# hugofloresgarcia/vampnet

Measured on NVIDIA H100. Metric: codec tokens/sec (coarse 12 steps + c2f 24 steps generate, T=768, 44.1 kHz), higher is better.
Workload: dtype bf16

## Files before the change

vampnet_b200/csrc/api.cu:

```cuda
#include <cuda_bf16.h>
#include <cudaTypedefs.h>

#include <cmath>
#include <cstdarg>
#include <cstdio>
#include <cstring>
#include <map>
#include <memory>
#include <string>
#include <tuple>
#include <vector>

#include "kernels.h"

namespace vnb {

static thread_local std::string g_err;
static thread_local std::string g_tmap_err;

static int fail(const char* fmt, ...) {
  char buf[1024];
  va_list ap;
  va_start(ap, fmt);
  vsnprintf(buf, sizeof(buf), fmt, ap);
// ... 27 lines not shown
  auto enc = get_encode();
  if (!enc) return false;
  cuuint64_t dims[2] = {cols, rows};
  cuuint64_t strides[1] = {cols * 2};
  cuuint32_t box[2] = {box_cols, box_rows};
  cuuint32_t estr[2] = {1, 1};
  CUresult r = enc(tm, CU_TENSOR_MAP_DATA_TYPE_BFLOAT16, 2, const_cast<void*>(base), dims, strides, box, estr,
                   CU_TENSOR_MAP_INTERLEAVE_NONE, CU_TENSOR_MAP_SWIZZLE_128B, CU_TENSOR_MAP_L2_PROMOTION_L2_256B,
                   CU_TENSOR_MAP_FLOAT_OOB_FILL_NONE);
  if (r != CUDA_SUCCESS) {
    char b[256];
    snprintf(b, sizeof(b), "cuTensorMapEncodeTiled(2d rows=%llu cols=%llu box=%ux%u) -> %d", (unsigned long long)rows,
             (unsigned long long)cols, box_rows, box_cols, (int)r);
    g_tmap_err = b;
    return false;
  }
  return true;
}
bool make_tmap_3d(CUtensorMap* tm, const void* base, uint64_t batch, uint64_t rows, uint64_t cols,
                  uint64_t pitch_elems, uint32_t box_rows, uint32_t box_cols) {
  auto enc = get_encode();
  if (!enc) return false;
  cuuint64_t dims[3] = {cols, rows, batch};
  cuuint64_t strides[2] = {pitch_elems * 2, rows * pitch_elems * 2};
  cuuint32_t box[3] = {box_cols, box_rows, 1};
  cuuint32_t estr[3] = {1, 1, 1};
  CUresult r = enc(tm, CU_TENSOR_MAP_DATA_TYPE_BFLOAT16, 3, const_cast<void*>(base), dims, strides, box, estr,
                   CU_TENSOR_MAP_INTERLEAVE_NONE, CU_TENSOR_MAP_SWIZZLE_128B, CU_TENSOR_MAP_L2_PROMOTION_L2_256B,
                   CU_TENSOR_MAP_FLOAT_OOB_FILL_NONE);
  if (r != CUDA_SUCCESS) {
    char b[256];
    snprintf(b, sizeof(b), "cuTensorMapEncodeTiled(3d batch=%llu rows=%llu cols=%llu pitch=%llu box=%ux%u) -> %d",
             (unsigned long long)batch, (unsigned long long)rows, (unsigned long long)cols,
             (unsigned long long)pitch_elems, box_rows, box_cols, (int)r);
    g_tmap_err = b;
    return false;
  }
  return true;
}

static bool make_gemm_plan(GemmPlan* p, int epi, const void* A, const void* W, int M, int N, int K, void* out,
                           void* out2, const float* bias, int T, int Tpad, const float* ss_in, int ss_parts,
                           float inv_d, float eps, void* out_bf16, float* ss_out) {
  if (N % 256 != 0 || K % 64 != 0 || M < 1) {
    g_tmap_err = "gemm: need N % 256 == 0 and K % 64 == 0";
    return false;
  }
  GemmArgs& a = p->args;
  a.M = M; a.N = N; a.K = K; a.epi = epi; a.out = out; a.out2 = out2; a.bias = bias;
  a.T = T; a.Tpad = Tpad; a.d2 = epi == VNB_EPI_QKV ? (N / 3) * 2 : 0;
  if (ss_in != nullptr) { a.ss_in = ss_in; a.ss_parts = ss_parts; a.inv_d = inv_d; a.eps = eps; }
  a.out_bf16 = reinterpret_cast<__nv_bfloat16*>(out_bf16); a.ss_out = ss_out;
  return make_tmap_2d(&p->tmA, A, M, K, 128, 64) && make_tmap_2d(&p->tmB, W, N, K, 256, 64) &&
         make_tmap_2d(&p->tmBh, W, N, K, 128, 64);
}

bool make_attn_plan(AttnPlan* p, const void* qk, const void* vT, void* out, const float* rel, int sat, int B, int T,
                    int Tpad, int H) {
  const int d = H * 64;
  p->out = out; p->rel = rel; p->sat = sat; p->B = B; p->T = T; p->Tpad = Tpad; p->H = H;
  return make_tmap_3d(&p->tmQ, qk, B, T, 2 * d, 2 * d, 128, 64) && make_tmap_3d(&p->tmK, qk, B, T, 2 * d, 2 * d, 64, 64) &&
         make_tmap_3d(&p->tmVT, vT, B, d, Tpad, Tpad, 64, 64);
}

struct DevBuf {
  void* p = nullptr;
  size_t n = 0;
  ~DevBuf() { if (p) cudaFree(p); }
  cudaError_t alloc(size_t bytes, bool zero = false) {
    n = bytes;
    cudaError_t e = cudaMalloc(&p, bytes ? bytes : 1);
    if (e == cudaSuccess && zero) e = cudaMemset(p, 0, bytes);
    return e;
  }
  template <class T> T* as() const { return reinterpret_cast<T*>(p); }
};

struct Variant {
  int steps = 0;
  bool has_mask = false;
  bool top_p = false;
  int gemm_pair = 0;
  bool fused = false;
  bool adapted = false;
  bool ragged = false;
  bool mixed_steps = false;
  bool split = false;
  bool operator<(const Variant& o) const {
    return std::tie(steps, has_mask, top_p, gemm_pair, fused, adapted, ragged, mixed_steps, split) <
           std::tie(o.steps, o.has_mask, o.top_p, o.gemm_pair, o.fused, o.adapted, o.ragged, o.mixed_steps, o.split);
  }
};

struct Workspace {
  int B = 0, T = 0, Tpad = 0, M = 0;
  unsigned long long last_use = 0;
  DevBuf x, y, qk, vT, att, h, logits, zcur, zorig, tokens, conf, n0, dyn, rowgrp, z_in, mask_in, z_out, ssA, ssB, embA,
      partials;
  DevBuf grp_adapter, lora_u;
  DevBuf frames;
  DevBuf live;
  int embKp = 0;
  int ss_parts = 0;
  std::vector<GemmPlan> qkv, wo, up, down;
  GemmPlan cls, emb;
  GemmPlan cls_sample;
  bool can_fuse = false;
// ... 1161 lines not shown
```

vampnet_b200/csrc/common.cuh:

```cuda
#pragma once
#include <cuda.h>
#include <cuda_bf16.h>
#include <cuda_runtime.h>
#include <stdint.h>
#include <stdio.h>

namespace vnb {

__device__ __forceinline__ uint32_t smem_u32(const void* p) {
  return static_cast<uint32_t>(__cvta_generic_to_shared(p));
}
__device__ __forceinline__ uint32_t lane_id() { return threadIdx.x & 31; }

__device__ __forceinline__ bool elect_one() {
  uint32_t pred = 0;
  asm volatile(
      "{\n\t.reg .pred P;\n\t.reg .b32 R;\n\t"
      "elect.sync R|P, 0xffffffff;\n\t"
      "selp.u32 %0, 1, 0, P;\n\t}"
      : "=r"(pred));
  return pred != 0;
}

__device__ __forceinline__ void mbar_init(uint64_t* bar, uint32_t count) {
// ... 121 lines not shown
  asm volatile(
      "{\n\t.reg .pred P;\n\t"
      "mbarrier.try_wait.parity.acquire.cluster.shared::cta.b64 P, [%1], %2, %3;\n\t"
      "selp.u32 %0, 1, 0, P;\n\t}"
      : "=r"(ok)
      : "r"(smem_u32(bar)), "r"(parity), "r"(100000u)
      : "memory");
  return ok != 0;
}
__device__ __forceinline__ void mbar_wait_cluster(uint64_t* bar, uint32_t parity) {
  if (mbar_try_wait_cluster(bar, parity)) return;
  const uint64_t t0 = global_timer_ns();
  while (!mbar_try_wait_cluster(bar, parity))
    if (global_timer_ns() - t0 > VNB_WAIT_TIMEOUT_NS) __trap();
}
__device__ __forceinline__ void tma_load_2d_mc(void* dst, const CUtensorMap* m, uint64_t* bar, int c0, int c1,
                                               uint16_t cta_mask) {
  asm volatile(
      "cp.async.bulk.tensor.2d.shared::cluster.global.mbarrier::complete_tx::bytes.multicast::cluster"
      " [%0], [%1, {%3, %4}], [%2], %5;"
      ::"r"(smem_u32(dst)), "l"(reinterpret_cast<uint64_t>(m)), "r"(smem_u32(bar)), "r"(c0), "r"(c1), "h"(cta_mask)
      : "memory");
}

__device__ __forceinline__ uint32_t pack_bf16x2(float lo, float hi) {
  __nv_bfloat162 v = __floats2bfloat162_rn(lo, hi);
  return *reinterpret_cast<uint32_t*>(&v);
}
__device__ __forceinline__ float fast_exp2(float x) {
  float y;
  asm volatile("ex2.approx.ftz.f32 %0, %1;" : "=f"(y) : "f"(x));
  return y;
}
__device__ __forceinline__ float lds_f32(uint32_t addr) {
  float v;
  asm volatile("ld.shared.f32 %0, [%1];" : "=f"(v) : "r"(addr));
  return v;
}
__device__ __forceinline__ void sts_f32(uint32_t addr, float v) {
  asm volatile("st.shared.f32 [%0], %1;" ::"r"(addr), "f"(v) : "memory");
}
__device__ __forceinline__ void sts_u32(uint32_t addr, uint32_t v) {
  asm volatile("st.shared.b32 [%0], %1;" ::"r"(addr), "r"(v) : "memory");
}
__device__ __forceinline__ float4 lds_f4(uint32_t addr) {
  float4 v;
  asm volatile("ld.shared.v4.f32 {%0, %1, %2, %3}, [%4];" : "=f"(v.x), "=f"(v.y), "=f"(v.z), "=f"(v.w) : "r"(addr));
  return v;
}
__device__ __forceinline__ uint2 lds_u2(uint32_t addr) {
  uint2 v;
  asm volatile("ld.shared.v2.b32 {%0, %1}, [%2];" : "=r"(v.x), "=r"(v.y) : "r"(addr));
  return v;
}
__device__ __forceinline__ void sts_f4(uint32_t addr, float4 v) {
  asm volatile("st.shared.v4.f32 [%0], {%1, %2, %3, %4};" ::"r"(addr), "f"(v.x), "f"(v.y), "f"(v.z), "f"(v.w)
               : "memory");
}
__device__ __forceinline__ void sts_v4(uint32_t addr, uint32_t a, uint32_t b, uint32_t c, uint32_t d) {
  asm volatile("st.shared.v4.b32 [%0], {%1, %2, %3, %4};" ::"r"(addr), "r"(a), "r"(b), "r"(c), "r"(d) : "memory");
}
__device__ __forceinline__ float warp_max(float v) {
#pragma unroll
  for (int o = 16; o > 0; o >>= 1) v = fmaxf(v, __shfl_xor_sync(0xffffffffu, v, o));
  return v;
}
__device__ __forceinline__ float warp_sum(float v) {
#pragma unroll
  for (int o = 16; o > 0; o >>= 1) v += __shfl_xor_sync(0xffffffffu, v, o);
  return v;
}

__device__ __forceinline__ void philox4x32_10(uint32_t c0, uint32_t c1, uint32_t c2, uint32_t c3, uint32_t k0,
                                              uint32_t k1, uint32_t (&out)[4]) {
#pragma unroll
  for (int r = 0; r < 10; ++r) {
    const uint32_t hi0 = __umulhi(0xD2511F53u, c0), lo0 = 0xD2511F53u * c0;
    const uint32_t hi1 = __umulhi(0xCD9E8D57u, c2), lo1 = 0xCD9E8D57u * c2;
    const uint32_t n0 = hi1 ^ c1 ^ k0, n2 = hi0 ^ c3 ^ k1;
    c0 = n0; c1 = lo1; c2 = n2; c3 = lo0;
    k0 += 0x9E3779B9u;
    k1 += 0xBB67AE85u;
  }
  out[0] = c0; out[1] = c1; out[2] = c2; out[3] = c3;
}
__device__ __forceinline__ float u01(uint32_t x) { return (static_cast<float>(x >> 9) + 0.5f) * 1.1920928955078125e-07f; }

}
```

vampnet_b200/csrc/gemm_wgmma.cu:

```cuda
#include <stdlib.h>

#include "common.cuh"
#include "kernels.h"
#include "wgmma.cuh"

#ifndef VNB_GEMM_PAIR_DEFAULT
#define VNB_GEMM_PAIR_DEFAULT false
#endif

namespace vnb {

constexpr int BM = 128, BN = 256, BK = 64, STAGES = 4;
constexpr int A_BYTES = BM * BK * 2;
constexpr int B_BYTES = BN * BK * 2;
constexpr int STAGE_BYTES = A_BYTES + B_BYTES;
constexpr int SBIAS_BYTES = BN * 4;
constexpr int RING_BYTES = STAGES * STAGE_BYTES;
constexpr int ACC_PITCH = BN + 1;
static_assert(BM * ACC_PITCH * 4 <= RING_BYTES, "the accumulator tile overlays the ring");
static_assert(BM * ACC_PITCH * 4 + 4 * BM + 16 + 32 * BM <= RING_BYTES, "the adapted epilogue's row table follows it");
constexpr int GEMM_SMEM = RING_BYTES + SBIAS_BYTES + 1024  + 256 ;
static_assert(GEMM_SMEM <= 227 * 1024, "H100: at most 227 KiB of shared memory per block");
constexpr int GEMM_THREADS = 256 + 32;
template <int EPI> constexpr int gemm_epi_warps() { return (EPI == VNB_EPI_RESID || EPI == VNB_EPI_SAMPLE) ? 8 : 4; }

__device__ __forceinline__ int live_rows(const GemmArgs& g) {
  if (g.live == nullptr) return g.M;
  const int r = __ldg(g.live) * g.T;
  return r < g.M ? r : g.M;
}

__device__ __forceinline__ float gelu_tanh(float x) {
  const float y = 0.7978845608028654f * (x + 0.044715f * x * x * x);
  const float e = __expf(2.0f * y);
  const float t = 1.0f - __fdividef(2.0f, 1.0f + e);
  return 0.5f * x * (1.0f + t);
}

__device__ __forceinline__ float row_scale(const GemmArgs& g, int row) {
  float rs = 1.0f;
  if (g.ss_in != nullptr && row < g.M) {
    float t = 0.f;
    for (int p = 0; p < g.ss_parts; ++p) t += __ldg(g.ss_in + static_cast<size_t>(p) * g.M + row);
    rs = rsqrtf(t * g.inv_d + g.eps);
  }
  return rs;
}


__device__ __forceinline__ float sumsq4(float x, float y, float z, float w) {
  return __fmaf_rn(w, w, __fmaf_rn(z, z, __fmaf_rn(y, y, __fmul_rn(x, x))));
}

template <int EPI>
__device__ __forceinline__ void prefetch_addend(const GemmArgs& g, int lane, int row_base, int col0, float4 (&add)[8]) {
  const int c4 = (lane & 7) * 4;
  const int r0 = row_base + (lane >> 3);
  if constexpr (EPI == VNB_EPI_RESID) {
    const float* base = reinterpret_cast<const float*>(g.out) + static_cast<size_t>(r0) * g.N + col0 + c4;
    const size_t step = static_cast<size_t>(4) * g.N;
#pragma unroll
    for (int it = 0; it < 8; ++it)
      add[it] = (r0 + it * 4 < g.M) ? __ldcg(reinterpret_cast<const float4*>(base + it * step))
                                    : make_float4(0.f, 0.f, 0.f, 0.f);
  } else {
    const float4 b4 = __ldg(reinterpret_cast<const float4*>(g.bias + col0 + c4));
#pragma unroll
    for (int it = 0; it < 8; ++it) add[it] = b4;
  }
}
template <bool FUSED>
__device__ __forceinline__ void drain_f32(const GemmArgs& g, uint32_t quad, float rs, int lane, int row_base, int n0,
                                          int c, const float4 (&add)[8], float (&ssacc)[8]) {
  const int c4 = (lane & 7) * 4;
  const int r0 = row_base + (lane >> 3);
  const int col0 = n0 + c * 32;
  float* const base = reinterpret_cast<float*>(g.out) + static_cast<size_t>(r0) * g.N + col0 + c4;
  const size_t step = static_cast<size_t>(4) * g.N;
#pragma unroll
  for (int it = 0; it < 8; ++it) {
    const int r = it * 4 + (lane >> 3);
    const float rsr = __shfl_sync(0xffffffffu, rs, r);
    const uint32_t sp = quad + 4u * (r * ACC_PITCH + c * 32 + c4);
    float4 a = make_float4(__fmul_rn(lds_f32(sp), rsr), __fmul_rn(lds_f32(sp + 4), rsr), __fmul_rn(lds_f32(sp + 8), rsr),
                           __fmul_rn(lds_f32(sp + 12), rsr));
    a.x = __fadd_rn(a.x, add[it].x); a.y = __fadd_rn(a.y, add[it].y);
    a.z = __fadd_rn(a.z, add[it].z); a.w = __fadd_rn(a.w, add[it].w);
    if (r0 + it * 4 < g.M) {
      *reinterpret_cast<float4*>(base + it * step) = a;
      if constexpr (FUSED) {
        uint2 w;
        w.x = pack_bf16x2(a.x, a.y);
        w.y = pack_bf16x2(a.z, a.w);
        *reinterpret_cast<uint2*>(g.out_bf16 + static_cast<size_t>(r0 + it * 4) * g.N + col0 + c4) = w;
        ssacc[it] = __fadd_rn(ssacc[it], sumsq4(a.x, a.y, a.z, a.w));
      }
    }
  }
}

template <bool GEGLU>
__device__ __forceinline__ void drain_bf16(__nv_bfloat16* out, int pitch, int M, uint32_t quad, float rs, int lane,
                                           int row_base, int tc, int oc) {
  const int c8 = (lane & 3) * 8;
#pragma unroll
  for (int it = 0; it < 4; ++it) {
    const int r = it * 8 + (lane >> 2);
    const float rsr = __shfl_sync(0xffffffffu, rs, r);
    const uint32_t sp = quad + 4u * (r * ACC_PITCH + tc + c8);
    float x[8];
#pragma unroll
    for (int k = 0; k < 8; ++k) {
      x[k] = lds_f32(sp + 4u * k) * rsr;
      if constexpr (GEGLU) x[k] = x[k] * gelu_tanh(lds_f32(sp + 4u * (128 + k)) * rsr);
    }
    const int row = row_base + r;
    if (row < M) {
      uint4 w;
      w.x = pack_bf16x2(x[0], x[1]);
      w.y = pack_bf16x2(x[2], x[3]);
      w.z = pack_bf16x2(x[4], x[5]);
      w.w = pack_bf16x2(x[6], x[7]);
      *reinterpret_cast<uint4*>(out + static_cast<size_t>(row) * pitch + oc + c8) = w;
    }
  }
}

__device__ __forceinline__ void acc_ld_x32(uint32_t addr, uint32_t (&v)[32]) {
#pragma unroll
  for (int j = 0; j < 32; ++j) v[j] = __float_as_uint(lds_f32(addr + 4u * j));
}

template <int EPI>
__device__ __forceinline__ void lora_update(const GemmArgs& g, uint8_t* scratch, uint32_t acc_tile, int m0, int n0) {
  int uoff = 0, brow0 = n0;
  if constexpr (EPI == VNB_EPI_QKV) {
    const int d = g.N / 3;
    if (n0 >= d && n0 < 2 * d) return;
    if (n0 >= 2 * d) { uoff = 8; brow0 = n0 - d; }
  }
  const AdapterRefs& L = g.lora;
  const int t = static_cast<int>(threadIdx.x);
  int32_t* sid = reinterpret_cast<int32_t*>(scratch);
  uint32_t* smask = reinterpret_cast<uint32_t*>(scratch + 4 * BM);
  float4* su = reinterpret_cast<float4*>(scratch + 4 * BM + 16);
  constexpr int R = EPI == VNB_EPI_QKV ? 16 : 8;
  if (t < BM) {
    const int m = m0 + t;
    const int id = m < g.M ? L.grp_adapter[L.rowgrp[m / L.rows_per_grp].group] : -1;
    sid[t] = id;
    if (id >= 0) {
      su[2 * t] = __ldg(reinterpret_cast<const float4*>(L.u + static_cast<size_t>(m) * R + uoff));
      su[2 * t + 1] = __ldg(reinterpret_cast<const float4*>(L.u + static_cast<size_t>(m) * R + uoff + 4));
    }
    uint32_t bits = 0;
    for (int a = 0; a < VNB_MAX_ADAPTERS; ++a) bits |= __ballot_sync(0xffffffffu, id == a) ? (1u << a) : 0u;
    if ((t & 31) == 0) smask[t >> 5] = bits;
  }
  asm volatile("bar.sync 1, 256;" ::: "memory");
  const uint32_t present = smask[0] | smask[1] | smask[2] | smask[3];
  const int nb = EPI == VNB_EPI_QKV ? 2 * (g.N / 3) : g.N;
  const int c0 = t & 63, rq = t >> 6;
  for (int a = 0; a < VNB_MAX_ADAPTERS; ++a) {
    if (!((present >> a) & 1u)) continue;
    const float* bp = L.table[a].b[L.slot] + (static_cast<size_t>(L.layer) * nb + brow0 + c0) * 8;
    float4 b0[4], b1[4];
#pragma unroll
    for (int j = 0; j < 4; ++j) {
      b0[j] = __ldg(reinterpret_cast<const float4*>(bp + 64 * 8 * j));
      b1[j] = __ldg(reinterpret_cast<const float4*>(bp + 64 * 8 * j + 4));
    }
#pragma unroll 4
    for (int i = 0; i < BM / 4; ++i) {
      const int r = rq + 4 * i;
      if (sid[r] != a) continue;
      const float4 ua = su[2 * r], ub = su[2 * r + 1];
      const uint32_t row_addr = acc_tile + 4u * (r * ACC_PITCH + c0);
#pragma unroll
      for (int j = 0; j < 4; ++j) {
        float s = __fmul_rn(ua.x, b0[j].x);
        s = __fmaf_rn(ua.y, b0[j].y, s); s = __fmaf_rn(ua.z, b0[j].z, s); s = __fmaf_rn(ua.w, b0[j].w, s);
        s = __fmaf_rn(ub.x, b1[j].x, s); s = __fmaf_rn(ub.y, b1[j].y, s); s = __fmaf_rn(ub.z, b1[j].z, s);
        s = __fmaf_rn(ub.w, b1[j].w, s);
        const uint32_t addr = row_addr + 4u * (64 * j);
        sts_f32(addr, __fadd_rn(lds_f32(addr), s));
      }
    }
  }
}

template <int NS, typename Release>
__device__ __forceinline__ void gemm_mainloop(float (&acc)[128], uint8_t* ring, uint64_t* full_bar, int num_kb, int wg,
                                              int& stage, uint32_t& phase, Release&& release) {
#pragma unroll
  for (int i = 0; i < 128; ++i) acc[i] = 0.f;
  for (int kb = 0; kb < num_kb; ++kb) {
    mbar_wait(&full_bar[stage], phase);
    const uint32_t sa = smem_u32(ring + stage * STAGE_BYTES) + wg * (64 * 128);
    const uint32_t sb = smem_u32(ring + stage * STAGE_BYTES + A_BYTES);
    wgmma_fence();
#pragma unroll
    for (int k = 0; k < BK / 16; ++k)
      wgmma_ss_n256(acc, wgmma_desc_sw128(sa + k * 32), wgmma_desc_sw128(sb + k * 32), 1u);
    wgmma_commit();
    wgmma_wait<1>();
    wgmma_fence_regs(acc);
    if (kb > 0) release(stage == 0 ? NS - 1 : stage - 1);
    if (++stage == NS) { stage = 0; phase ^= 1; }
  }
  wgmma_wait<0>();
  wgmma_fence_regs(acc);
  if (num_kb > 0) release(stage == 0 ? NS - 1 : stage - 1);
}

template <int EPI, bool PAIR, bool ADAPT = false, bool SPLIT = false>
__global__ void __launch_bounds__(GEMM_THREADS, 1)
gemm_wgmma_kernel(const __grid_constant__ CUtensorMap tmA, const __grid_constant__ CUtensorMap tmB,
                  const GemmArgs g) {
  extern __shared__ uint8_t smem_raw[];
  uint8_t* smem = reinterpret_cast<uint8_t*>((reinterpret_cast<uintptr_t>(smem_raw) + 1023) & ~uintptr_t(1023));
  float* sbias_all = reinterpret_cast<float*>(smem + RING_BYTES);
  uint64_t* full_bar = reinterpret_cast<uint64_t*>(smem + RING_BYTES + SBIAS_BYTES);
  uint64_t* empty_bar = full_bar + STAGES;

  const int warp = threadIdx.x >> 5;
  const int lane = threadIdx.x & 31;
  const uint32_t rank = PAIR ? cluster_ctarank() : 0u;
  const int tile = PAIR ? static_cast<int>(blockIdx.x >> 1) : static_cast<int>(blockIdx.x);
  constexpr int TM = PAIR ? 2 * BM : BM;
  const int num_n = g.N / BN;
  const int num_kb = g.K / BK;
  const int m0 = (tile / num_n) * TM + static_cast<int>(rank) * BM;
  const int n0 = (tile % num_n) * BN;
  if (g.live != nullptr && (tile / num_n) * TM >= live_rows(g)) return;

  if (warp == 8 && lane == 0) {
    tma_prefetch_desc(&tmA);
    tma_prefetch_desc(&tmB);
    for (int s = 0; s < STAGES; ++s) {
      mbar_init(&full_bar[s], 1);
      mbar_init(&empty_bar[s], 8 * (PAIR ? 2 : 1));
    }
    mbar_fence_init();
  }
  if constexpr (PAIR) cluster_sync_all();
  else __syncthreads();

  if (warp == 8) {
    if (lane == 0) {
      int stage = 0;
      uint32_t phase = 0;
      for (int kb = 0; kb < num_kb; ++kb) {
        if constexpr (PAIR) mbar_wait_cluster(&empty_bar[stage], phase ^ 1);
        else mbar_wait(&empty_bar[stage], phase ^ 1);
        uint8_t* sa = smem + stage * STAGE_BYTES;
        uint8_t* sb = sa + A_BYTES;
// ... 122 lines not shown
            uint32_t v[32];
            acc_ld_x32(t_strip + 4u * (c * 32), v);
#pragma unroll
            for (int j4 = 0; j4 < 8; ++j4) {
              const float4 b4 = lds_f4(sb4 + 16u * (c * 8 + j4));
              const float bj[4] = {b4.x, b4.y, b4.z, b4.w};
#pragma unroll
              for (int j = 0; j < 4; ++j) {
                const float x = __fadd_rn(__fmul_rn(__uint_as_float(v[j4 * 4 + j]), rs), bj[j]);
                ssum += fast_exp2(__fmaf_rn(x, c1, c0));
              }
            }
          }
          int cand = am;
          float xc = mx;
          if (do_sample) {
            uint32_t r4[4];
            philox4x32_10(static_cast<uint32_t>(t_idx * Cp + cp), static_cast<uint32_t>(b_idx - rg.first),
                          static_cast<uint32_t>(dyn.step), 0u, dyn.seed_lo, dyn.seed_hi, r4);
            const float target = u01(r4[1]) * ssum;
            float run = 0.f;
            int found = -1;
#pragma unroll 1
            for (int c = 0; c < 4; ++c) {
              uint32_t v[32];
              acc_ld_x32(t_strip + 4u * (c * 32), v);
#pragma unroll
              for (int j4 = 0; j4 < 8; ++j4) {
                const float4 b4 = lds_f4(sb4 + 16u * (c * 8 + j4));
                const float bj[4] = {b4.x, b4.y, b4.z, b4.w};
#pragma unroll
                for (int j = 0; j < 4; ++j) {
                  const float x = __fadd_rn(__fmul_rn(__uint_as_float(v[j4 * 4 + j]), rs), bj[j]);
                  run += fast_exp2(__fmaf_rn(x, c1, c0));
                  if (run > target && found < 0) { found = c * 32 + j4 * 4 + j; xc = x; }
                }
              }
            }
            if (found >= 0) cand = found;
            else xc = mx;
          }
          if (active)
            g.partials[(static_cast<size_t>(row) * Cp + cp) * (g.V >> 7) + (v0 >> 7)] =
                make_float4(mx, ssum, xc, __uint_as_float(static_cast<uint32_t>(v0 + cand) |
                                                          (static_cast<uint32_t>(v0 + am) << 16)));
        }
      } else if constexpr (EPI == VNB_EPI_RESID || EPI == VNB_EPI_BIAS_F32) {
        const bool fused_out = g.out_bf16 != nullptr;
        constexpr int CSTEP = kWide ? 2 : 1;
        float ssacc[8];
#pragma unroll
        for (int i = 0; i < 8; ++i) ssacc[i] = 0.f;
        auto process = [&](int c, const float4 (&add)[8]) {
          if (fused_out) drain_f32<true>(g, qaddr, rs, lane, row_base, n0, c, add, ssacc);
          else drain_f32<false>(g, qaddr, rs, lane, row_base, n0, c, add, ssacc);
        };
        float4 addA[8], addB[8];
        prefetch_addend<EPI>(g, lane, row_base, n0 + half * 32, addA);
#pragma unroll 1
        for (int c = half; c < BN / 32; c += 2 * CSTEP) {
          prefetch_addend<EPI>(g, lane, row_base, n0 + (c + CSTEP) * 32, addB);
          process(c, addA);
          if (c + 2 * CSTEP < BN / 32) prefetch_addend<EPI>(g, lane, row_base, n0 + (c + 2 * CSTEP) * 32, addA);
          process(c + CSTEP, addB);
        }
        if (fused_out) {
#pragma unroll
          for (int it = 0; it < 8; ++it) {
            float v = ssacc[it];
            v += __shfl_xor_sync(0xffffffffu, v, 1);
            v += __shfl_xor_sync(0xffffffffu, v, 2);
            v += __shfl_xor_sync(0xffffffffu, v, 4);
            const int rr = row_base + it * 4 + (lane >> 3);
            const int part = (n0 / BN) * (kWide ? 2 : 1) + half;
            if ((lane & 7) == 0 && rr < g.M) g.ss_out[static_cast<size_t>(part) * g.M + rr] = v;
          }
        }
      } else {
#pragma unroll 1
        for (int c = 0; c < BN / 32; ++c) {
          const int col0 = n0 + c * 32;
          if constexpr (EPI == VNB_EPI_QKV) {
            if (col0 >= g.d2) {
              uint32_t v[32];
              acc_ld_x32(t_addr + 4u * (c * 32), v);
              if (row_ok) {
                const int d = g.N - g.d2;
                __nv_bfloat16* o = reinterpret_cast<__nv_bfloat16*>(g.out2) +
                                   (static_cast<size_t>(b_idx) * d + (col0 - g.d2)) * g.Tpad + t_idx;
                const bool pad = g.frames != nullptr && t_idx >= __ldg(g.frames + b_idx);
#pragma unroll
                for (int j = 0; j < 32; ++j)
                  o[static_cast<size_t>(j) * g.Tpad] =
                      pad ? __float2bfloat16_rn(0.f) : __float2bfloat16_rn(__uint_as_float(v[j]) * rs);
              }
              continue;
            }
          }
          drain_bf16<false>(reinterpret_cast<__nv_bfloat16*>(g.out), EPI == VNB_EPI_BF16 ? g.N : g.d2, g.M, qaddr, rs, lane,
                            row_base, c * 32, col0);
        }
      }
    }
  }
  if constexpr (PAIR) cluster_sync_all();
}

constexpr int PERS_EPI_WARPS = 3;
// ... 138 lines not shown
        for (int u = e; u < BM / 2; u += PERS_EPI_WARPS) {
          const int rr = 2 * u + (lane >> 4);
          const float4 v = lds_f4(stage_tile + stage_off<256>(rr, 4 * (lane & 15)));
          if (m0 + rr < g.M)
            *reinterpret_cast<float4*>(out + static_cast<size_t>(m0 + rr) * pitch + (n0 >> 1) + 8 * (lane & 15)) = v;
        }
      } else if (n0 < g.d2) {
#pragma unroll 4
        for (int rr = e; rr < BM; rr += PERS_EPI_WARPS) {
          const float4 v = lds_f4(stage_tile + stage_off<512>(rr, 4 * lane));
          if (m0 + rr < g.M)
            *reinterpret_cast<float4*>(out + static_cast<size_t>(m0 + rr) * pitch + n0 + 8 * lane) = v;
        }
      } else {
        const int d = g.N - g.d2;
        uint16_t* const vt = reinterpret_cast<uint16_t*>(g.out2) + static_cast<size_t>(n0 - g.d2) * g.Tpad;
        size_t off[4];
        bool ok[4];
        int bk[4];
        uint32_t keep[2] = {0xffffffffu, 0xffffffffu};
#pragma unroll
        for (int k = 0; k < 4; ++k) {
          const int m = m0 + 4 * lane + k;
          bk[k] = m / g.T;
          const int t = m - bk[k] * g.T;
          ok[k] = m < g.M;
          off[k] = static_cast<size_t>(bk[k]) * d * g.Tpad + t;
          if (ok[k] && g.frames != nullptr && t >= __ldg(g.frames + bk[k])) keep[k >> 1] &= (k & 1) ? 0xffffu : 0xffff0000u;
        }
        const bool wide = ok[3] && bk[3] == bk[0] && (off[0] & 3) == 0 && (g.Tpad & 3) == 0 &&
                          (reinterpret_cast<uintptr_t>(g.out2) & 7) == 0;
#pragma unroll 2
        for (int c = e; c < BN; c += PERS_EPI_WARPS) {
          uint2 v = lds_u2(stage_tile + stage_off<256>(c, 2 * lane));
          v.x &= keep[0];
          v.y &= keep[1];
          uint16_t* const o = vt + static_cast<size_t>(c) * g.Tpad;
          if (wide) {
            *reinterpret_cast<uint2*>(o + off[0]) = v;
          } else {
#pragma unroll
            for (int k = 0; k < 4; ++k) {
              const uint32_t w = k < 2 ? v.x : v.y;
              if (ok[k]) o[off[k]] = static_cast<uint16_t>((k & 1) ? (w >> 16) : w);
            }
          }
        }
      }
      row_scales(tile + gridDim.x);
    }
  }
}

static int g_gemm_pair = -1;
void set_gemm_pair(int on) { g_gemm_pair = on ? 1 : 0; }
static bool gemm_pair_enabled() {
  if (g_gemm_pair < 0) {
    const char* e = getenv("VNB_GEMM_PAIR");
    g_gemm_pair = e != nullptr ? (e[0] == '1') : (VNB_GEMM_PAIR_DEFAULT ? 1 : 0);
  }
  return g_gemm_pair == 1;
}
int get_gemm_pair() { return gemm_pair_enabled() ? 1 : 0; }

static int g_max_clusters[6][64];
template <int EPI>
static cudaError_t init_epi() {
  static PerDeviceOnce once;
  int dev;
  if (!once.need(&dev)) return cudaSuccess;
  cudaError_t e = cudaFuncSetAttribute(gemm_wgmma_kernel<EPI, false>, cudaFuncAttributeMaxDynamicSharedMemorySize, GEMM_SMEM);
  if (e != cudaSuccess) return e;
  e = cudaFuncSetAttribute(gemm_wgmma_kernel<EPI, true>, cudaFuncAttributeMaxDynamicSharedMemorySize, GEMM_SMEM);
  if (e != cudaSuccess) return e;
  if constexpr (EPI == VNB_EPI_QKV || EPI == VNB_EPI_RESID || EPI == VNB_EPI_GEGLU) {
    e = cudaFuncSetAttribute(gemm_wgmma_kernel<EPI, false, true>, cudaFuncAttributeMaxDynamicSharedMemorySize, GEMM_SMEM);
    if (e != cudaSuccess) return e;
    e = cudaFuncSetAttribute(gemm_wgmma_kernel<EPI, true, true>, cudaFuncAttributeMaxDynamicSharedMemorySize, GEMM_SMEM);
    if (e != cudaSuccess) return e;
  }
  if constexpr (EPI == VNB_EPI_GEGLU || EPI == VNB_EPI_QKV) {
    e = cudaFuncSetAttribute(gemm_persistent_kernel<EPI>, cudaFuncAttributeMaxDynamicSharedMemorySize, pers_smem<EPI>());
    if (e != cudaSuccess) return e;
  }
  if constexpr (EPI == VNB_EPI_SAMPLE) {
    e = cudaFuncSetAttribute(gemm_wgmma_kernel<EPI, false, false, true>, cudaFuncAttributeMaxDynamicSharedMemorySize,
                             GEMM_SMEM);
    if (e != cudaSuccess) return e;
    e = cudaFuncSetAttribute(gemm_wgmma_kernel<EPI, true, false, true>, cudaFuncAttributeMaxDynamicSharedMemorySize,
                             GEMM_SMEM);
    if (e != cudaSuccess) return e;
  }
  cudaLaunchConfig_t q = {};
  q.gridDim = dim3(2 * device_sm_count());
  q.blockDim = dim3(GEMM_THREADS);
  q.dynamicSmemBytes = GEMM_SMEM;
  cudaLaunchAttribute qa[1];
  qa[0].id = cudaLaunchAttributeClusterDimension;
  qa[0].val.clusterDim.x = 2; qa[0].val.clusterDim.y = 1; qa[0].val.clusterDim.z = 1;
  q.attrs = qa; q.numAttrs = 1;
  int n = 0;
  e = cudaOccupancyMaxActiveClusters(&n, gemm_wgmma_kernel<EPI, true>, &q);
  if (e != cudaSuccess || n <= 0) { (void)cudaGetLastError(); n = device_sm_count() / 2; }
  if (dev >= 0 && dev < 64) g_max_clusters[EPI][dev] = n;
  once.mark(dev);
  return cudaSuccess;
}
cudaError_t prepare_gemm() {
  cudaError_t e;
  if ((e = init_epi<VNB_EPI_BF16>()) != cudaSuccess) return e;
  if ((e = init_epi<VNB_EPI_QKV>()) != cudaSuccess) return e;
  if ((e = init_epi<VNB_EPI_RESID>()) != cudaSuccess) return e;
  if ((e = init_epi<VNB_EPI_GEGLU>()) != cudaSuccess) return e;
  if ((e = init_epi<VNB_EPI_BIAS_F32>()) != cudaSuccess) return e;
  return init_epi<VNB_EPI_SAMPLE>();
}

int get_gemm_max_clusters() {
  int dev = 0;
  cudaGetDevice(&dev);
  if (prepare_gemm() != cudaSuccess || dev < 0 || dev >= 64) return 0;
  return g_max_clusters[VNB_EPI_RESID][dev];
}

template <int EPI, bool ADAPT = false, bool SPLIT = false>
static cudaError_t launch_epi(const GemmPlan& p, const GemmArgs& g, cudaStream_t st) {
  cudaError_t e = init_epi<EPI>();
  if (e != cudaSuccess) return e;
  if (gemm_pair_enabled()) {
    const int clusters = ((g.M + 2 * BM - 1) / (2 * BM)) * (g.N / BN);
    cudaLaunchConfig_t cfg = {};
    cfg.gridDim = dim3(2 * clusters);
    cfg.blockDim = dim3(GEMM_THREADS);
    cfg.dynamicSmemBytes = GEMM_SMEM;
    cfg.stream = st;
    cudaLaunchAttribute attr[1];
    attr[0].id = cudaLaunchAttributeClusterDimension;
    attr[0].val.clusterDim.x = 2; attr[0].val.clusterDim.y = 1; attr[0].val.clusterDim.z = 1;
    cfg.attrs = attr; cfg.numAttrs = 1;
    return cudaLaunchKernelEx(&cfg, gemm_wgmma_kernel<EPI, true, ADAPT, SPLIT>, p.tmA, p.tmBh, g);
  }
  const int tiles = ((g.M + BM - 1) / BM) * (g.N / BN);
  if constexpr ((EPI == VNB_EPI_GEGLU || EPI == VNB_EPI_QKV) && !ADAPT) {
    const int grid = tiles < device_sm_count() ? tiles : device_sm_count();
    gemm_persistent_kernel<EPI><<<grid, PERS_THREADS, pers_smem<EPI>(), st>>>(p.tmA, p.tmB, g);
    return cudaGetLastError();
  }
  gemm_wgmma_kernel<EPI, false, ADAPT, SPLIT><<<tiles, GEMM_THREADS, GEMM_SMEM, st>>>(p.tmA, p.tmB, g);
  return cudaGetLastError();
}

cudaError_t launch_gemm(const GemmPlan& p, cudaStream_t st) {
  GemmArgs g = p.args;
  if (g.epi != VNB_EPI_QKV) g.frames = nullptr;
  if (g.lora.table != nullptr) {
    if (!g.lora.grp_adapter || !g.lora.rowgrp || !g.lora.u || g.lora.rows_per_grp < 1) return cudaErrorInvalidValue;
    switch (g.epi) {
      case VNB_EPI_QKV: return launch_epi<VNB_EPI_QKV, true>(p, g, st);
      case VNB_EPI_RESID: return launch_epi<VNB_EPI_RESID, true>(p, g, st);
      case VNB_EPI_GEGLU: return launch_epi<VNB_EPI_GEGLU, true>(p, g, st);
      default: return cudaErrorInvalidValue;
    }
  }
  switch (g.epi) {
    case VNB_EPI_BF16: return launch_epi<VNB_EPI_BF16>(p, g, st);
    case VNB_EPI_QKV: return launch_epi<VNB_EPI_QKV>(p, g, st);
    case VNB_EPI_RESID: return launch_epi<VNB_EPI_RESID>(p, g, st);
    case VNB_EPI_GEGLU: return launch_epi<VNB_EPI_GEGLU>(p, g, st);
    case VNB_EPI_BIAS_F32: return launch_epi<VNB_EPI_BIAS_F32>(p, g, st);
    case VNB_EPI_SAMPLE:
      if (!g.zcur || !g.dyn || !g.rowgrp || !g.partials || !g.bias || g.V % 128 != 0 || g.V > 1024) return cudaErrorInvalidValue;
      if (p.sample_split) {
        if (!g.out) return cudaErrorInvalidValue;
        return launch_epi<VNB_EPI_SAMPLE, false, true>(p, g, st);
      }
      return launch_epi<VNB_EPI_SAMPLE>(p, g, st);
    default: return cudaErrorInvalidValue;
  }
}

__global__ void gemm_ref_kernel(const __nv_bfloat16* A, const __nv_bfloat16* W, int M, int N, int K, float* out) {
  const int n = blockIdx.x * blockDim.x + threadIdx.x;
  const int m = blockIdx.y;
  if (n >= N || m >= M) return;
  float acc = 0.f;
  for (int k = 0; k < K; ++k)
    acc += __bfloat162float(A[static_cast<size_t>(m) * K + k]) * __bfloat162float(W[static_cast<size_t>(n) * K + k]);
  out[static_cast<size_t>(m) * N + n] = acc;
}
cudaError_t launch_gemm_ref(const void* A, const void* W, int M, int N, int K, float* out, cudaStream_t st) {
  dim3 grid((N + 127) / 128, M);
  gemm_ref_kernel<<<grid, 128, 0, st>>>(reinterpret_cast<const __nv_bfloat16*>(A),
                                        reinterpret_cast<const __nv_bfloat16*>(W), M, N, K, out);
  return cudaGetLastError();
}

}
```

vampnet_b200/csrc/kernels.h:

```cpp
#pragma once
#include <cuda.h>
#include <cuda_bf16.h>
#include <cuda_runtime.h>
#include <stdint.h>

#include "../../include/vampnet_b200.h"

namespace vnb {

struct PerDeviceOnce {
  unsigned long long done = 0;
  bool need(int* dev_out) {
    int dev = 0;
    cudaGetDevice(&dev);
    *dev_out = dev;
    return dev >= 64 || !((done >> dev) & 1ull);
  }
  void mark(int dev) { if (dev < 64) done |= 1ull << dev; }
};
inline int device_sm_count() {
  static int sms[64] = {0};
  int dev = 0;
  cudaGetDevice(&dev);
  if (dev >= 64) { int n = 0; cudaDeviceGetAttribute(&n, cudaDevAttrMultiProcessorCount, dev); return n; }
// ... 8 lines not shown
bool make_tmap_3d(CUtensorMap* tm, const void* base, uint64_t batch, uint64_t rows, uint64_t cols,
                  uint64_t pitch_elems, uint32_t box_rows, uint32_t box_cols);
const char* tmap_error();
}
extern "C" int32_t vnb_set_error_cuda(const char* what, int32_t cuda_error);
namespace vnb {

struct SampleDyn;
struct RowGroup {
  int32_t group, first;
};

enum { LORA_QKV = 0, LORA_WO, LORA_W1, LORA_W2, LORA_SLOTS };
struct AdapterDev {
  const float* a[LORA_SLOTS];
  const float* b[LORA_SLOTS];
};
struct AdapterRefs {
  const AdapterDev* table = nullptr;
  const int32_t* grp_adapter = nullptr;
  const RowGroup* rowgrp = nullptr;
  int rows_per_grp = 1;
  int slot = 0, layer = 0;
  float* u = nullptr;
};
cudaError_t launch_lora_down(const void* y, int M, int K, const AdapterRefs& r, const int32_t* live, int T,
                             cudaStream_t st);

struct GemmArgs {
  int M, N, K;
  int epi;
  void* out;
  void* out2;
  const float* bias;
  int T, Tpad;
  int d2;
  __nv_bfloat16* out_bf16;
  float* ss_out;
  const float* ss_in;
  int ss_parts;
  float inv_d, eps;
  const int32_t* zcur;
  const SampleDyn* dyn;
  const RowGroup* rowgrp;
  float4* partials;
  int C, ncc, V, mask_token;
  AdapterRefs lora;
  const int32_t* frames;
  const int32_t* live;
};
struct GemmPlan {
  CUtensorMap tmA, tmB;
  CUtensorMap tmBh;
  bool sample_split = false;
  GemmArgs args{};
};
cudaError_t launch_gemm(const GemmPlan& p, cudaStream_t st);
cudaError_t prepare_gemm();
void set_gemm_pair(int on);
int get_gemm_pair();
int get_gemm_max_clusters();
cudaError_t launch_gemm_ref(const void* A, const void* W, int M, int N, int K, float* out, cudaStream_t st);

struct AttnPlan {
  CUtensorMap tmQ;
  CUtensorMap tmK;
  CUtensorMap tmVT;
  void* out = nullptr;
  const float* rel = nullptr;
  const int32_t* frames = nullptr;
  const int32_t* live = nullptr;
  int sat = 0, B = 0, T = 0, Tpad = 0, H = 0;
};
bool make_attn_plan(AttnPlan* p, const void* qk, const void* vT, void* out, const float* rel, int sat, int B, int T,
                    int Tpad, int H);
cudaError_t launch_attention(const AttnPlan& p, cudaStream_t st);

cudaError_t launch_embed_gather(const int32_t* codes_btc, const float* latents, const float* table, void* A, int M, int T,
                                int C, int V1, int K, int Kp, float* ss, int zero_from, int ss_parts,
                                const int32_t* live, cudaStream_t st);

cudaError_t launch_gen_init(const int64_t* z, const int32_t* mask, int32_t* zcur, int32_t* zorig, int32_t* n0,
                            const RowGroup* rowgrp, int n_groups, int B, int C, int T, int ncc, int mask_token,
                            cudaStream_t st);
cudaError_t launch_gen_finish(const int32_t* tokens, const int32_t* zorig, int64_t* out, int B, int C, int T, int ncc,
                              cudaStream_t st);

struct SampleDyn {
  float inv_temp, gamma, temp_eff;
  int do_sample, is_last, step;
  uint32_t seed_lo, seed_hi;
  float top_p;
};
struct SampleArgs {
  const float* logits;
  int32_t* zcur;
  const int32_t* zorig;
  int32_t* tokens;
  float* conf;
  const int32_t* n0;
  const RowGroup* rowgrp;
  int B, T, C, ncc, V, mask_token;
  const int32_t* live = nullptr;
};
cudaError_t launch_sample_step_dev(const SampleArgs& a, const SampleDyn* dyn_dev, cudaStream_t st, bool use_top_p);
cudaError_t launch_sample_combine_dev(const SampleArgs& a, const void* partials, const SampleDyn* dyn_dev, cudaStream_t st);
// ... 70 lines not shown
```

Baseline: 294,800.

## Add persistent warp-specialized residual GEMM with BN=128 tiles and overlapped epilogue

```diff
diff --git a/vampnet_b200/csrc/api.cu b/vampnet_b200/csrc/api.cu
--- a/vampnet_b200/csrc/api.cu
+++ b/vampnet_b200/csrc/api.cu
@@ -103,7 +103,7 @@
   if (ss_in != nullptr) { a.ss_in = ss_in; a.ss_parts = ss_parts; a.inv_d = inv_d; a.eps = eps; }
   a.out_bf16 = reinterpret_cast<__nv_bfloat16*>(out_bf16); a.ss_out = ss_out;
   return make_tmap_2d(&p->tmA, A, M, K, 128, 64) && make_tmap_2d(&p->tmB, W, N, K, 256, 64) &&
-         make_tmap_2d(&p->tmBh, W, N, K, 128, 64);
+         make_tmap_2d(&p->tmBh, W, N, K, 128, 64) && make_tmap_2d(&p->tmB32, W, N, K, 32, 64);
 }
 
 bool make_attn_plan(AttnPlan* p, const void* qk, const void* vT, void* out, const float* rel, int sat, int B, int T,
diff --git a/vampnet_b200/csrc/common.cuh b/vampnet_b200/csrc/common.cuh
--- a/vampnet_b200/csrc/common.cuh
+++ b/vampnet_b200/csrc/common.cuh
@@ -197,6 +197,9 @@
   uint2 v;
   asm volatile("ld.shared.v2.b32 {%0, %1}, [%2];" : "=r"(v.x), "=r"(v.y) : "r"(addr));
   return v;
+}
+__device__ __forceinline__ void sts_f2(uint32_t addr, float x, float y) {
+  asm volatile("st.shared.v2.f32 [%0], {%1, %2};" ::"r"(addr), "f"(x), "f"(y) : "memory");
 }
 __device__ __forceinline__ void sts_f4(uint32_t addr, float4 v) {
   asm volatile("st.shared.v4.f32 [%0], {%1, %2, %3, %4};" ::"r"(addr), "f"(v.x), "f"(v.y), "f"(v.z), "f"(v.w)
diff --git a/vampnet_b200/csrc/gemm_wgmma.cu b/vampnet_b200/csrc/gemm_wgmma.cu
--- a/vampnet_b200/csrc/gemm_wgmma.cu
+++ b/vampnet_b200/csrc/gemm_wgmma.cu
@@ -52,6 +52,10 @@
   return __fmaf_rn(w, w, __fmaf_rn(z, z, __fmaf_rn(y, y, __fmul_rn(x, x))));
 }
 
+__device__ __forceinline__ uint32_t resid_off(int r, int w) {
+  return static_cast<uint32_t>(r * 512 + (((w >> 2) ^ ((r & 3) << 1)) << 4) + ((w & 3) << 2));
+}
+
 template <int EPI>
 __device__ __forceinline__ void prefetch_addend(const GemmArgs& g, int lane, int row_base, int col0, float4 (&add)[8]) {
   const int c4 = (lane & 7) * 4;
@@ -69,21 +73,26 @@
     for (int it = 0; it < 8; ++it) add[it] = b4;
   }
 }
-template <bool FUSED>
-__device__ __forceinline__ void drain_f32(const GemmArgs& g, uint32_t quad, float rs, int lane, int row_base, int n0,
-                                          int c, const float4 (&add)[8], float (&ssacc)[8]) {
+template <bool FUSED, bool SWZ = false>
+__device__ __forceinline__ void drain_f32(const GemmArgs& g, uint32_t quad, float rs, int lane, int row_base, int c,
+                                          int col0, const float4 (&add)[8], float (&ssacc)[8]) {
   const int c4 = (lane & 7) * 4;
   const int r0 = row_base + (lane >> 3);
-  const int col0 = n0 + c * 32;
   float* const base = reinterpret_cast<float*>(g.out) + static_cast<size_t>(r0) * g.N + col0 + c4;
   const size_t step = static_cast<size_t>(4) * g.N;
 #pragma unroll
   for (int it = 0; it < 8; ++it) {
     const int r = it * 4 + (lane >> 3);
     const float rsr = __shfl_sync(0xffffffffu, rs, r);
-    const uint32_t sp = quad + 4u * (r * ACC_PITCH + c * 32 + c4);
-    float4 a = make_float4(__fmul_rn(lds_f32(sp), rsr), __fmul_rn(lds_f32(sp + 4), rsr), __fmul_rn(lds_f32(sp + 8), rsr),
-                           __fmul_rn(lds_f32(sp + 12), rsr));
+    float4 a;
+    if constexpr (SWZ) {
+      a = lds_f4(quad + resid_off(r, c * 32 + c4));
+      a = make_float4(__fmul_rn(a.x, rsr), __fmul_rn(a.y, rsr), __fmul_rn(a.z, rsr), __fmul_rn(a.w, rsr));
+    } else {
+      const uint32_t sp = quad + 4u * (r * ACC_PITCH + c * 32 + c4);
+      a = make_float4(__fmul_rn(lds_f32(sp), rsr), __fmul_rn(lds_f32(sp + 4), rsr), __fmul_rn(lds_f32(sp + 8), rsr),
+                      __fmul_rn(lds_f32(sp + 12), rsr));
+    }
     a.x = __fadd_rn(a.x, add[it].x); a.y = __fadd_rn(a.y, add[it].y);
     a.z = __fadd_rn(a.z, add[it].z); a.w = __fadd_rn(a.w, add[it].w);
     if (r0 + it * 4 < g.M) {
@@ -189,19 +198,23 @@
   }
 }
 
-template <int NS, typename Release>
-__device__ __forceinline__ void gemm_mainloop(float (&acc)[128], uint8_t* ring, uint64_t* full_bar, int num_kb, int wg,
+template <int NS, int NACC, typename Release>
+__device__ __forceinline__ void gemm_mainloop(float (&acc)[NACC], uint8_t* ring, uint64_t* full_bar, int num_kb, int wg,
                                               int& stage, uint32_t& phase, Release&& release) {
-#pragma unroll
-  for (int i = 0; i < 128; ++i) acc[i] = 0.f;
+  static_assert(NACC == 128 || NACC == 64, "m64n256k16 or m64n128k16");
+  constexpr int SB = A_BYTES + 2 * NACC * BK * 2;
+#pragma unroll
+  for (int i = 0; i < NACC; ++i) acc[i] = 0.f;
   for (int kb = 0; kb < num_kb; ++kb) {
     mbar_wait(&full_bar[stage], phase);
-    const uint32_t sa = smem_u32(ring + stage * STAGE_BYTES) + wg * (64 * 128);
-    const uint32_t sb = smem_u32(ring + stage * STAGE_BYTES + A_BYTES);
+    const uint32_t sa = smem_u32(ring + stage * SB) + wg * (64 * 128);
+    const uint32_t sb = smem_u32(ring + stage * SB + A_BYTES);
     wgmma_fence();
 #pragma unroll
-    for (int k = 0; k < BK / 16; ++k)
-      wgmma_ss_n256(acc, wgmma_desc_sw128(sa + k * 32), wgmma_desc_sw128(sb + k * 32), 1u);
+    for (int k = 0; k < BK / 16; ++k) {
+      if constexpr (NACC == 128) wgmma_ss_n256(acc, wgmma_desc_sw128(sa + k * 32), wgmma_desc_sw128(sb + k * 32), 1u);
+      else wgmma_ss_n128(acc, wgmma_desc_sw128(sa + k * 32), wgmma_desc_sw128(sb + k * 32), 1u);
+    }
     wgmma_commit();
     wgmma_wait<1>();
     wgmma_fence_regs(acc);
@@ -430,8 +443,8 @@
 #pragma unroll
         for (int i = 0; i < 8; ++i) ssacc[i] = 0.f;
         auto process = [&](int c, const float4 (&add)[8]) {
-          if (fused_out) drain_f32<true>(g, qaddr, rs, lane, row_base, n0, c, add, ssacc);
-          else drain_f32<false>(g, qaddr, rs, lane, row_base, n0, c, add, ssacc);
+          if (fused_out) drain_f32<true>(g, qaddr, rs, lane, row_base, c, n0 + c * 32, add, ssacc);
+          else drain_f32<false>(g, qaddr, rs, lane, row_base, c, n0 + c * 32, add, ssacc);
         };
         float4 addA[8], addB[8];
         prefetch_addend<EPI>(g, lane, row_base, n0 + half * 32, addA);
@@ -676,6 +689,132 @@
   }
 }
 
+constexpr int RES_BN = 128;
+constexpr int RES_STAGES = 5;
+constexpr int RES_STAGE_BYTES = A_BYTES + RES_BN * BK * 2;
+constexpr int RES_OUT_BYTES = BM * RES_BN * 4;
+constexpr int RES_EPI_WARPS = 4;
+constexpr int RES_THREADS = 256 + 32 * RES_EPI_WARPS + 32;
+constexpr int RES_SMEM = RES_STAGES * RES_STAGE_BYTES + RES_OUT_BYTES + 1024  + 128 ;
+static_assert(RES_SMEM <= 227 * 1024, "H100: at most 227 KiB of shared memory per block");
+static_assert((2 * RES_STAGES + 2) * 8 <= 128, "the barriers fit their slot");
+
+__global__ void __launch_bounds__(RES_THREADS, 1)
+gemm_persistent_resid_kernel(const __grid_constant__ CUtensorMap tmA, const __grid_constant__ CUtensorMap tmB32,
+                             const GemmArgs g) {
+  constexpr int NS = RES_STAGES;
+  constexpr int RING = NS * RES_STAGE_BYTES;
+  extern __shared__ uint8_t smem_raw[];
+  uint8_t* smem = reinterpret_cast<uint8_t*>((reinterpret_cast<uintptr_t>(smem_raw) + 1023) & ~uintptr_t(1023));
+  const uint32_t stage_tile = smem_u32(smem + RING);
+  uint64_t* full_bar = reinterpret_cast<uint64_t*>(smem + RING + RES_OUT_BYTES);
+  uint64_t* empty_bar = full_bar + NS;
+  uint64_t* out_full = empty_bar + NS;
+  uint64_t* out_free = out_full + 1;
+
+  const int warp = threadIdx.x >> 5;
+  const int lane = threadIdx.x & 31;
+  const int num_t = 2 * (g.N / BN);
+  const int num_kb = g.K / BK;
+  const int tiles = ((live_rows(g) + BM - 1) / BM) * num_t;
+  constexpr int kProducer = 8 + RES_EPI_WARPS;
+
+  if (warp == kProducer && lane == 0) {
+    tma_prefetch_desc(&tmA);
+    tma_prefetch_desc(&tmB32);
+    for (int s = 0; s < NS; ++s) {
+      mbar_init(&full_bar[s], 1);
+      mbar_init(&empty_bar[s], 8);
+    }
+    mbar_init(out_full, 256);
+    mbar_init(out_free, 32 * RES_EPI_WARPS);
+    mbar_fence_init();
+  }
+  __syncthreads();
+
+  if (warp == kProducer) {
+    if (lane == 0) {
+      int stage = 0;
+      uint32_t phase = 0;
+      for (int tile = blockIdx.x; tile < tiles; tile += gridDim.x) {
+        const int m0 = (tile / num_t) * BM, nt = tile % num_t;
+        const int c0 = (nt >> 1) * BN + (nt & 1) * 32;
+        for (int kb = 0; kb < num_kb; ++kb) {
+          mbar_wait(&empty_bar[stage], phase ^ 1);
+          uint8_t* sa = smem + stage * RES_STAGE_BYTES;
+          mbar_expect_tx(&full_bar[stage], RES_STAGE_BYTES);
+          tma_load_2d(sa, &tmA, &full_bar[stage], kb * BK, m0);
+#pragma unroll
+          for (int j = 0; j < 4; ++j)
+            tma_load_2d(sa + A_BYTES + j * (32 * BK * 2), &tmB32, &full_bar[stage], kb * BK, c0 + 64 * j);
+          if (++stage == NS) { stage = 0; phase ^= 1; }
+        }
+      }
+    }
+    __syncwarp();
+  } else if (warp < 8) {
+    int stage = 0;
+    uint32_t phase = 0;
+    uint32_t it = 0;
+    const int r = (warp >> 2) * 64 + (warp & 3) * 16 + (lane >> 2);
+    for (int tile = blockIdx.x; tile < tiles; tile += gridDim.x, ++it) {
+      float acc[64];
+      gemm_mainloop<NS>(acc, smem, full_bar, num_kb, warp >> 2, stage, phase, [&](int s) {
+        if (lane == 0) mbar_arrive(&empty_bar[s]);
+      });
+      mbar_wait(out_free, (it & 1u) ^ 1u);
+#pragma unroll
+      for (int i = 0; i < 16; ++i) {
+        const int w = 8 * i + 2 * (lane & 3);
+        sts_f2(stage_tile + resid_off(r, w), acc[4 * i], acc[4 * i + 1]);
+        sts_f2(stage_tile + resid_off(r + 8, w), acc[4 * i + 2], acc[4 * i + 3]);
+      }
+      mbar_arrive(out_full);
+    }
+  } else {
+    const int quad = warp - 8;
+    const uint32_t qaddr = stage_tile + 512u * (32 * quad);
+    const bool fused_out = g.out_bf16 != nullptr;
+    uint32_t it = 0;
+    for (int tile = blockIdx.x; tile < tiles; tile += gridDim.x, ++it) {
+      const int m0 = (tile / num_t) * BM, nt = tile % num_t;
+      const int n0 = (nt >> 1) * BN, half = nt & 1;
+      const int row_base = m0 + quad * 32;
+      const float rs = row_scale(g, row_base + lane);
+      float ssacc[8];
+#pragma unroll
+      for (int i = 0; i < 8; ++i) ssacc[i] = 0.f;
+      auto process = [&](int j, const float4 (&add)[8]) {
+        if (fused_out) drain_f32<true, true>(g, qaddr, rs, lane, row_base, j, n0 + (2 * j + half) * 32, add, ssacc);
+        else drain_f32<false, true>(g, qaddr, rs, lane, row_base, j, n0 + (2 * j + half) * 32, add, ssacc);
+      };
+      float4 addA[8], addB[8];
+      prefetch_addend<VNB_EPI_RESID>(g, lane, row_base, n0 + half * 32, addA);
+      mbar_wait(out_full, it & 1u);
+#pragma unroll 1
+      for (int j = 0; j < 4; j += 2) {
+        prefetch_addend<VNB_EPI_RESID>(g, lane, row_base, n0 + (2 * j + 2 + half) * 32, addB);
+        process(j, addA);
+        if (j + 2 < 4) prefetch_addend<VNB_EPI_RESID>(g, lane, row_base, n0 + (2 * j + 4 + half) * 32, addA);
+        process(j + 1, addB);
+      }
+      mbar_arrive(out_free);
+      if (fused_out) {
+#pragma unroll
+        for (int i = 0; i < 8; ++i) {
+          float v = ssacc[i];
+          v += __shfl_xor_sync(0xffffffffu, v, 1);
+          v += __shfl_xor_sync(0xffffffffu, v, 2);
+          v += __shfl_xor_sync(0xffffffffu, v, 4);
+          const int rr = row_base + i * 4 + (lane >> 3);
+          const int part = (n0 / BN) * 2 + half;
+          if ((lane & 7) == 0 && rr < g.M) g.ss_out[static_cast<size_t>(part) * g.M + rr] = v;
+        }
+      }
+    }
+  }
+}
+
 static int g_gemm_pair = -1;
 void set_gemm_pair(int on) { g_gemm_pair = on ? 1 : 0; }
 static bool gemm_pair_enabled() {
@@ -705,6 +844,10 @@
   }
   if constexpr (EPI == VNB_EPI_GEGLU || EPI == VNB_EPI_QKV) {
     e = cudaFuncSetAttribute(gemm_persistent_kernel<EPI>, cudaFuncAttributeMaxDynamicSharedMemorySize, pers_smem<EPI>());
+    if (e != cudaSuccess) return e;
+  }
+  if constexpr (EPI == VNB_EPI_RESID) {
+    e = cudaFuncSetAttribute(gemm_persistent_resid_kernel, cudaFuncAttributeMaxDynamicSharedMemorySize, RES_SMEM);
     if (e != cudaSuccess) return e;
   }
   if constexpr (EPI == VNB_EPI_SAMPLE) {
@@ -770,6 +913,12 @@
     gemm_persistent_kernel<EPI><<<grid, PERS_THREADS, pers_smem<EPI>(), st>>>(p.tmA, p.tmB, g);
     return cudaGetLastError();
   }
+  if constexpr (EPI == VNB_EPI_RESID && !ADAPT) {
+    const int res_tiles = 2 * tiles;
+    const int grid = res_tiles < device_sm_count() ? res_tiles : device_sm_count();
+    gemm_persistent_resid_kernel<<<grid, RES_THREADS, RES_SMEM, st>>>(p.tmA, p.tmB32, g);
+    return cudaGetLastError();
+  }
   gemm_wgmma_kernel<EPI, false, ADAPT, SPLIT><<<tiles, GEMM_THREADS, GEMM_SMEM, st>>>(p.tmA, p.tmB, g);
   return cudaGetLastError();
 }
diff --git a/vampnet_b200/csrc/kernels.h b/vampnet_b200/csrc/kernels.h
--- a/vampnet_b200/csrc/kernels.h
+++ b/vampnet_b200/csrc/kernels.h
@@ -84,6 +84,7 @@
 struct GemmPlan {
   CUtensorMap tmA, tmB;
   CUtensorMap tmBh;
+  CUtensorMap tmB32;
   bool sample_split = false;
   GemmArgs args{};
 };
```

Result: no change. 295,900, median of 6 (+0.4%).
